# theEricMa/TriplaneTurbo

Measured on AMD Instinct MI355X. Metric: rendered rays/sec (fwd+bwd) at 256x256 rays x 128 samples, higher is better.
Workload: dtype f32 (fp32-grade: exact 3-piece fp16 operand split, 6 x v_mfma_f32_32x32x16_f16 per k-step, fp32 accumulation)

## Files before the change

### triplaneturbo_amd/csrc/tt_backward.hip

```cpp
#include "tt_backward_common.h"

struct BwdGeoParams {
    const float* packed;
    MlpPtrs w;
    const float* rays_o;
    const float* rays_d;
    const float* t_starts;
    const float* t_ends;
    tt_render_cfg cfg;
    TileGeom geom;
    long long n_items;
    int* queue;
    const float* ws;
    int n_copies;
    float* grad_packed;
    MlpGradPtrs grads;
    unsigned long long* phase_cycles;
};

#define GEO_SCRATCH_FLOATS (2 * 64 * XS)
#define GOFF_W1T LDS_GEO_FLOATS
#define GOFF_W2T (GOFF_W1T + IMG16_FLOATS(32, 64))
#define LDS_GEO16_FLOATS (GOFF_W2T + IMG16_FLOATS(64, 64))
#define GLO_W1 LDS_GEO16_FLOATS
#define GLO_W2 (GLO_W1 + LO16_FLOATS(64, 32))
#define GLO_W1T (GLO_W2 + LO16_FLOATS(64, 64))
#define GLO_W2T (GLO_W1T + LO16_FLOATS(32, 64))
#define LDS_GEO3_FLOATS (GLO_W2T + LO16_FLOATS(64, 64))
template <int PREC>
struct GeoWFloats {
    static constexpr int value = PREC == PREC_S3 ? LDS_GEO3_FLOATS : LDS_GEO16_FLOATS;
};

template <int PREC, bool WG16, bool STATS = false>
__global__ __launch_bounds__(256, 1) void k_decode_bwd_geo(BwdGeoParams p) {
    constexpr bool EXACT = PREC == PREC_F32;
    constexpr int NT = PrecNT<PREC>::value, WF = GeoWFloats<PREC>::value;
    __shared__ __attribute__((aligned(16))) float L[WF + 4 * (GEO_SCRATCH_FLOATS + SCATTER_TAG_INTS)];
    {
        MlpPtrs w = p.w;
        stage_weights<PREC, 64, 32>(L + OFF_W1, L + GLO_W1, w.w1);
        stage_weights<PREC, 64, 64>(L + OFF_W2, L + GLO_W2, w.w2);
        lds_load_matrix(L + OFF_W3, w.w3, 1, 64, 64);
        stage_weights_t<PREC, 64, 32>(L + GOFF_W1T, L + GLO_W1T, w.w1);
        stage_weights_t<PREC, 64, 64>(L + GOFF_W2T, L + GLO_W2T, w.w2);
    }
    const tt_render_cfg& cfg = p.cfg;
    float sA1 = 1.f, sU = 1.f, sA2 = 1.f, sV = 1.f;
    if (WG16) {
        const unsigned* bnd = reinterpret_cast<const unsigned*>(p.queue) + TT_SLOT_BOUNDS;
        const float Pm = __builtin_bit_cast(float, bnd[TT_BOUND_PLANES]), Sb = __builtin_bit_cast(float, bnd[TT_BOUND_UP0]),
                    Gb = __builtin_bit_cast(float, bnd[TT_BOUND_UP1]);
        unsigned* word = reinterpret_cast<unsigned*>(L + WF);
        const int t = threadIdx.x;
        float w1row = 0.f, a1col = 0.f, w3abs = 0.f;
        if (t < 64) {
            for (int c = 0; c < 32; ++c) w1row += __builtin_fabsf(p.w.w1[t * 32 + c]);
            for (int r = 0; r < 64; ++r) a1col += __builtin_fabsf(p.w.w2[r * 64 + t]) * __builtin_fabsf(p.w.w3[r]);
            w3abs = __builtin_fabsf(p.w.w3[t]);
        }
        const float W1max = block_max(w1row, word), A1max = block_max(a1col, word), A2max = block_max(w3abs, word);
        const float jsum = (0.5f * cfg.plane_w + 0.5f * cfg.plane_h) / cfg.radius;
        const float Fmax = 3.f * Pm, H1max = W1max * Fmax;
        const float Umax = Fmax * (Sb + 2.f * jsum * Gb), QBmax = Fmax * 2.f * jsum * Gb;
        const float Vmax = Sb * H1max + W1max * QBmax;
        sA1 = wg16_scale(A1max);
        sU = wg16_scale(Umax);
        sA2 = wg16_scale(A2max);
        sV = wg16_scale(Vmax);
    }
    const TileGeom& tg = p.geom;
    const int lane = threadIdx.x & 63, i = lane & 31, hi = lane >> 5, wave_in_blk = threadIdx.x >> 6;
    float* Xs = L + WF + wave_in_blk * (GEO_SCRATCH_FLOATS + SCATTER_TAG_INTS);
    float* Ys = Xs + 64 * XS;
    int* tags = reinterpret_cast<int*>(Ys + 64 * XS);
    scatter_init_tags(tags, lane);
    __syncthreads();
    const int S = cfg.n_samples;
    ItemQueue iq = item_queue(p.queue, tg.n_blocks, tg.n_chunks, tg.unit);
    const int H = cfg.plane_h, W = cfg.plane_w;
    const size_t HW = (size_t)H * W;
    const size_t plane_stride = 6 * HW * TT_C;
    const float ju = 0.5f * W / cfg.radius, jv = 0.5f * H / cfg.radius;
    float* const grad_out =
        p.grad_packed + (size_t)(blockIdx.x % (unsigned)p.n_copies) * cfg.n_prompts * plane_stride;
    const unsigned grad_bytes =
        TT_DBG(cfg.flags, TT_DBG_NO_ATOMICS) ? 0u : (unsigned)(cfg.n_prompts * plane_stride * sizeof(float));

    const TileStats st = STATS ? tile_stats(cfg.stats) : TileStats{nullptr};
    f32x16 accW1[2][1] = {{ZERO16}, {ZERO16}};
    f32x16 accW2[2][2] = {{ZERO16, ZERO16}, {ZERO16, ZERO16}};
    float accw3 = 0.f;
#ifdef TT_TUNING
    unsigned long long ph_acc[20] = {0, 0, 0, 0, 0, 0, 0, 0, 0, 0, 0, 0, 0, 0, 0, 0, 0, 0, 0, 0};
    unsigned long long ph_t = __builtin_amdgcn_s_memtime();
#endif

#pragma nounroll
    for (;;) {
        long long b;
        int ck;
        if (!item_pop(iq, tg.order, tg.n_chunks, b, ck)) break;
        if (b >= tg.n_blocks) continue;
        bool ray_ok;
        const long long ray = tile_ray(tg, b, i, ray_ok);
        const float ray_okf = tt_opaque(ray_ok ? 1.f : 0.f);
        const int ks = i % tg.sb;
        const int view = (int)(ray / cfg.rays_per_view);
        const size_t pofs = (size_t)(view / cfg.views_per_prompt) * plane_stride;
        const float ox = p.rays_o[ray * 3 + 0], oy = p.rays_o[ray * 3 + 1], oz = p.rays_o[ray * 3 + 2];
        const float dx = p.rays_d ? p.rays_d[ray * 3 + 0] : 0.f, dy = p.rays_d ? p.rays_d[ray * 3 + 1] : 0.f,
                    dz = p.rays_d ? p.rays_d[ray * 3 + 2] : 0.f;
        const int s_end = (ck + 1) * tg.chunk < S ? (ck + 1) * tg.chunk : S;
        struct StepIn {
            f32x4 up;
            float ts, te;
        };
        auto load_step = [&](int sb0) {
            StepIn r;
            const int si = sb0 + ks;
            const long long sidx = ray * S + (si < S ? si : S - 1);
            r.up = *reinterpret_cast<const f32x4*>(p.ws + sidx * 4);
            r.ts = p.rays_d ? p.t_starts[sidx] : 0.f;
            r.te = p.rays_d ? p.t_ends[sidx] : 0.f;
            return r;
        };
        StepIn in = load_step(ck * tg.chunk), in_next;
#pragma nounroll
        for (int sb0 = ck * tg.chunk; sb0 < s_end; sb0 += tg.sb, in = in_next) {
            in_next = load_step(sb0 + tg.sb);
            const int si = sb0 + ks;
            const bool rvalid = ray_ok && si < s_end;
            const float vf = ray_okf * (si < s_end ? 1.f : 0.f);
            const float sbar = in.up[0] * vf, gbx = in.up[1] * vf, gby = in.up[2] * vf, gbz = in.up[3] * vf;
            tile_stat(st, TT_STAT_VISITED);
            TT_PHASE(0);
            if (!__any(!((__builtin_fabsf(sbar) + __builtin_fabsf(gbx)) + (__builtin_fabsf(gby) + __builtin_fabsf(gbz)) <=
                         cfg.skip_eps_geo)))
                continue;
            float tm, px, py, pz;
            sample_position(ox, oy, oz, dx, dy, dz, in.ts, in.te, tm, px, py, pz);
            const float X = scale_coord(px, cfg.radius), Y = scale_coord(py, cfg.radius),
                        Z = scale_coord(pz, cfg.radius);
            float f[16], u[16];
            unsigned pmask;
            const bool any = __any(gather_geo_bwd_c(p.packed, (unsigned)(pofs / TT_C), H, W, X, Y, Z, rvalid, sbar, gbx,
                                                    gby, gbz, ju, jv, lane, Xs, f, u, pmask,
                                                    tile_stat_ptr(st, TT_STAT_INBOUNDS)));
            TT_PHASE(1);
            if (!any) continue;
            const bool one = single_plane(pmask);
            tile_stat_executed(st, one);
            float h1[32], h2[32], a2[32], a1[32], q[16], u1, u2;
            mvx<PREC, 64, 32, true>(L + OFF_W1, L + GLO_W1, f, h1, i, hi, 1.f, &u1);
#pragma unroll
            for (int r = 0; r < 32; ++r) h1[r] = fmaxf(h1[r], 0.f);
            mvx<PREC, 64, 64, true>(L + OFF_W2, L + GLO_W2, h1, h2, i, hi, u1, &u2);
#pragma unroll
            for (int r = 0; r < 32; ++r) h2[r] = fmaxf(h2[r], 0.f);
#pragma unroll
            for (int g = 0; g < 8; ++g) {
                f32x4 w3 = *reinterpret_cast<const f32x4*>(L + OFF_W3 + 8 * g + 4 * hi);
#pragma unroll
                for (int e2 = 0; e2 < 4; ++e2) a2[4 * g + e2] = h2[4 * g + e2] > 0.f ? w3[e2] : 0.f;
            }
            Split16<64, PAIR_SEQ, NT> a2s, a1s;
            float ua1 = 1.f;
            if (WG16) {
                split16_vec<64, PAIR_SEQ, NT>(a2, sA2, a2s);
                mv16_pre<64, 64, true, NT>(L + GOFF_W2T, a2s, 1.f / sA2, a1, i, hi, &ua1, L + GLO_W2T);
            } else {
                mvtx_copy<PREC, 64, 64, 64>(L + GOFF_W2T, L + GLO_W2T, L + OFF_W2, a2, a1, i, hi);
            }
#pragma unroll
            for (int r = 0; r < 32; ++r) a1[r] = h1[r] > 0.f ? a1[r] : 0.f;
            if (WG16) {
                split16_vec<64, PAIR_SEQ, NT>(a1, sA1 * ua1, a1s);
                mv16_pre<32, 64, false, NT>(L + GOFF_W1T, a1s, 1.f / sA1, q, i, hi, nullptr, L + GLO_W1T);
            } else {
                mvtx_copy<PREC, 32, 64, 32>(L + GOFF_W1T, L + GLO_W1T, L + OFF_W1, a1, q, i, hi);
            }
            TT_PHASE(3);
            {
                float qb[16];
#pragma unroll
                for (int r = 0; r < 16; ++r) qb[r] = fmaf(-sbar, f[r], u[r]);
                const bool region = WG16 ? true : cfg.flags >= 0;
                const bool do_wgrad = region && !TT_DBG(cfg.flags, TT_DBG_NO_WGRAD);
                if (do_wgrad) {
                    if (WG16) {
                        stage_rows16_pre<64>(Xs, a1s, i, hi);
                        stage_rows16<32>(Ys, u, i, hi, sU);
                        wgrad16<64, 32>(accW1, Xs, Ys, i, hi);
                    } else {
                        stage_rows<64>(Xs, a1, i, hi);
                        stage_rows<32>(Ys, u, i, hi);
                        wgrad<64, 32>(accW1, Xs, Ys, i, hi);
                    }
                }
                TT_PHASE(7);
                float t1[32];
                mvx<PREC, 64, 32>(L + OFF_W1, L + GLO_W1, qb, t1, i, hi);
#pragma unroll
                for (int r = 0; r < 32; ++r) t1[r] = h1[r] > 0.f ? t1[r] : 0.f;
                float v[32];
#pragma unroll
                for (int r = 0; r < 32; ++r) v[r] = fmaf(sbar * u1, h1[r], t1[r]);
                TT_PHASE(4);
                if (do_wgrad) {
                    if (WG16) {
                        stage_rows16_pre<64>(Xs, a2s, i, hi);
                        stage_rows16<64>(Ys, v, i, hi, sV);
                        wgrad16<64, 64>(accW2, Xs, Ys, i, hi);
                    } else {
                        stage_rows<64>(Xs, a2, i, hi);
                        stage_rows<64>(Ys, v, i, hi);
                        wgrad<64, 64>(accW2, Xs, Ys, i, hi);
                    }
                }
                TT_PHASE(8);
                float t2[32];
                mvx<PREC, 64, 64>(L + OFF_W2, L + GLO_W2, t1, t2, i, hi);
#pragma unroll
                for (int r = 0; r < 32; ++r) t2[r] = fmaf(sbar * u2, h2[r], h2[r] > 0.f ? t2[r] : 0.f);
                stage_rows<64>(Xs, t2, i, hi);
                accw3 += rowsum32(Xs, lane);
                TT_PHASE(5);
                if (region && !TT_DBG(cfg.flags, TT_DBG_NO_SCATTER)) {
                    scatter_clear<EXACT>(Xs, lane);
                    float* Qs = Xs + SCATTER_M_FLOATS;
                    TT_PHASE(9);
                    const int tex0 = (int)(pofs / TT_C);
                    auto prep = [&](int pl, PlaneRefs& refs) {
                        Corners c;
                        float coef[4];
                        geo_corner_coefs(pl, H, W, X, Y, Z, rvalid, sbar, gbx, gby, gbz, ju, jv, c, coef);
                        int aoff[4];
#pragma unroll
                        for (int q4 = 0; q4 < 4; ++q4) aoff[q4] = tex0 + (int)(pl * HW) + c.off[q4];
                        refs = plane_refs<!EXACT>(coef, aoff, c.hs, hi);
#pragma unroll
                        for (int r = 0; r < 16; ++r) Qs[i * 33 + LIDX(r, hi)] = q[r] * refs.qs;
                    };
#ifdef TT_TUNING
                    unsigned long long* const sc_st = ph_acc + 14;
#else
                    unsigned long long* const sc_st = nullptr;
#endif
                    if (one)
                        scatter_one_plane<EXACT>(grad_out, grad_bytes, Qs, Xs, tags, Qs + 32 * 33, i, hi,
                                                 single_plane_index(pmask), prep, sc_st);
                    else
                        scatter_planes<EXACT>(grad_out, grad_bytes, Qs, Xs, tags, Qs + 32 * 33, i, hi, prep, sc_st);
                    TT_PHASE(10);
                }
            }
        }
    }
#ifdef TT_TUNING
    TT_PHASE(11);
    if (p.phase_cycles && lane == 0)
        for (int k = 0; k < 20; ++k) atomicAdd(p.phase_cycles + 20 + k, ph_acc[k]);
#endif
    __syncthreads();
    int parity = 0;
    flush_wgrad_reduced<64, 32>(L, parity, accW1, p.grads.w1, wave_in_blk, lane, 1.f / sA1, 1.f / sU);
    flush_wgrad_reduced<64, 64>(L, parity, accW2, p.grads.w2, wave_in_blk, lane, 1.f / sA2, 1.f / sV);
    atomicAdd(p.grads.w3 + lane, accw3);
    tile_stats_flush(st);
}

#ifdef TT_TUNING
unsigned long long* g_phase_cycles = nullptr;
extern "C" int tt_tuning_phase_cycles(unsigned long long* out40) {
    if (!g_phase_cycles) {
        if (hipMalloc((void**)&g_phase_cycles, 40 * sizeof(unsigned long long)) != hipSuccess) return -4;
        if (hipMemset(g_phase_cycles, 0, 40 * sizeof(unsigned long long)) != hipSuccess) return -4;
    }
    if (hipDeviceSynchronize() != hipSuccess) return -4;
    if (out40 && hipMemcpy(out40, g_phase_cycles, 40 * sizeof(unsigned long long), hipMemcpyDeviceToHost) != hipSuccess)
        return -4;
    return hipMemset(g_phase_cycles, 0, 40 * sizeof(unsigned long long)) == hipSuccess ? 0 : -4;
}
#endif
static void launch_bwd_geo(const BwdGeoParams& p0, long long blocks, hipStream_t s) {
    BwdGeoParams p = p0;
#ifdef TT_TUNING
    p.phase_cycles = g_phase_cycles;
#else
    p.phase_cycles = nullptr;
#endif
    if (use_wg16(p.cfg)) {
        unsigned* bnd = reinterpret_cast<unsigned*>(p.queue) + TT_SLOT_BOUNDS;
        launch_planes_bound(p.packed, p.cfg, 0, bnd + TT_BOUND_PLANES, s);
        const long long n = p.cfg.n_rays * p.cfg.n_samples;
        hipLaunchKernelGGL(k_absmax4, dim3(absmax_blocks(n), 1), dim3(256), 0, s, reinterpret_cast<const f32x4*>(p.ws), n, n,
                           bnd + TT_BOUND_UP0, bnd + TT_BOUND_UP1);
    }
    tt_dispatch_prec(tt_prec_of_r(p.cfg.flags), [&](auto P) {
        constexpr int PREC = decltype(P)::value;
        constexpr bool WG16 = PREC != PREC_F32;
        if (p.cfg.stats)
            hipLaunchKernelGGL((k_decode_bwd_geo<PREC, WG16, true>), dim3((unsigned)blocks), dim3(256), 0, s, p);
        else
            hipLaunchKernelGGL((k_decode_bwd_geo<PREC, WG16>), dim3((unsigned)blocks), dim3(256), 0, s, p);
    });
}

extern "C" int tt_render_bwd_geo(const float* packed, const tt_mlp_weights* w, const float* rays_o,
                                 const float* rays_d, const float* t_starts, const float* t_ends,
                                 const tt_render_cfg* cfg, const float* opacity, const float* depth,
                                 const float* trans, const float* sdf, const float* sdf_grad, const float* features,
                                 const float* g_opacity, const float* g_depth, const float* g_rgb_fg,
                                 const float* g_z_variance, const float* g_normal_acc, const float* g_weights,
                                 const float* g_sdf, const float* g_sdf_grad, float* g_inv_std_rays, float* workspace,
                                 float* grad_packed, const tt_mlp_grads* grads, void* stream) {
    int st = tt_validate_cfg(cfg);
    if (st != TT_OK) return st;
    if (!packed || !w || !rays_o || !rays_d || !t_starts || !t_ends || !opacity || !depth || !trans || !sdf ||
        !sdf_grad || !features || !workspace || !grad_packed || !grads)
        return TT_ERR_BAD_ARG;
    if (!w->w1 || !w->w2 || !w->w3 || !grads->w1 || !grads->w2 || !grads->w3) return TT_ERR_BAD_ARG;
    if (grad_buffer_too_large(cfg)) return TT_ERR_UNSUPPORTED;
    int cus = tt_num_cus();
    if (cus <= 0) return TT_ERR_DEVICE;
    hipStream_t s = (hipStream_t)stream;
    st = tt_launch_march_bwd(rays_d, t_starts, t_ends, cfg, sdf, sdf_grad, features, trans, opacity, depth, g_opacity,
                             g_depth, g_rgb_fg, g_z_variance, g_normal_acc, g_weights, g_sdf, g_sdf_grad, g_inv_std_rays,
                             workspace, s);
    if (st != TT_OK) return st;
    BwdGeoParams p;
    tt_fill_rays(p, packed, w, rays_o, rays_d, t_starts, t_ends, *cfg);
    p.cfg.flags |= debug_flags();
    p.ws = workspace;
    p.grad_packed = grad_packed;
    p.n_copies = cfg->grad_copies > 0 ? cfg->grad_copies : 1;
    p.grads = to_gptrs(grads);
    st = tt_plan_queue(cfg, 4LL * cus, s, &p.geom, &p.n_items, &p.queue);
    if (st != TT_OK) return st;
    launch_bwd_geo(p, tt_persistent_blocks(p.n_items, cus, 4), s);
    return tt_check_launch();
}

__global__ void k_interleave_ws(const float* __restrict__ g_sdf, const float* __restrict__ g_sdf_grad,
                                float* __restrict__ ws, long long n) {
    const long long i = (long long)blockIdx.x * blockDim.x + threadIdx.x;
    if (i >= n) return;
    f32x4 o = {g_sdf ? g_sdf[i] : 0.f, g_sdf_grad ? g_sdf_grad[i * 3 + 0] : 0.f,
               g_sdf_grad ? g_sdf_grad[i * 3 + 1] : 0.f, g_sdf_grad ? g_sdf_grad[i * 3 + 2] : 0.f};
    *reinterpret_cast<f32x4*>(ws + i * 4) = o;
}

extern "C" int tt_points_bwd_geo(const float* packed, const tt_mlp_weights* w, const float* points, int32_t n_batch,
                                 int64_t n_points, int32_t n_prompts, int32_t views_per_prompt, int32_t plane_h,
                                 int32_t plane_w, float radius, float sdf_bias_radius, int32_t flags,
                                 const float* g_sdf, const float* g_sdf_grad, float* workspace, float* grad_packed,
                                 const tt_mlp_grads* grads, void* stream) {
    tt_render_cfg cfg;
    int st = points_cfg(&cfg, n_batch, n_points, n_prompts, views_per_prompt, plane_h, plane_w, radius,
                        sdf_bias_radius, 1, flags);
    if (st != TT_OK) return st;
    if (grad_buffer_too_large(&cfg)) return TT_ERR_UNSUPPORTED;
    if (!packed || !w || !points || !workspace || !grad_packed || !grads || (!g_sdf && !g_sdf_grad))
        return TT_ERR_BAD_ARG;
    if (!w->w1 || !w->w2 || !w->w3 || !grads->w1 || !grads->w2 || !grads->w3) return TT_ERR_BAD_ARG;
    int cus = tt_num_cus();
    if (cus <= 0) return TT_ERR_DEVICE;
    hipStream_t s = (hipStream_t)stream;
    const long long n = cfg.n_rays;
    hipLaunchKernelGGL(k_interleave_ws, dim3((unsigned)((n + 255) / 256)), dim3(256), 0, s, g_sdf, g_sdf_grad,
                       workspace, n);
    st = tt_check_launch();
    if (st != TT_OK) return st;
    BwdGeoParams p;
    tt_fill_rays(p, packed, w, points, nullptr, nullptr, nullptr, cfg);
    p.ws = workspace;
    p.grad_packed = grad_packed;
    p.n_copies = 1;
    p.grads = to_gptrs(grads);
    st = tt_plan_queue(&cfg, 4LL * cus, s, &p.geom, &p.n_items, &p.queue);
    if (st != TT_OK) return st;
    launch_bwd_geo(p, tt_persistent_blocks(p.n_items, cus, 4), s);
    return tt_check_launch();
}
```

### triplaneturbo_amd/csrc/tt_backward_common.h

```cpp
#pragma once
#include "tt_device.h"
#include "tt_mfma16.h"
#include "tt_alpha.h"
#include "tt_launch.h"
#include <type_traits>

typedef int i32x4 __attribute__((ext_vector_type(4)));

#ifdef TT_TUNING
#define TT_PHASE(k)                                              \
    do {                                                         \
        __builtin_amdgcn_sched_barrier(0);                       \
        const unsigned long long t_now = __builtin_amdgcn_s_memtime(); \
        ph_acc[k] += t_now - ph_t;                               \
        ph_t = t_now;                                            \
        __builtin_amdgcn_sched_barrier(0);                       \
    } while (0)
#else
#define TT_PHASE(k) \
    do {            \
    } while (0)
#endif
#define XS 36

template <int N>
__device__ __forceinline__ void stage_rows(float* S, const float (&v)[N / 2], int j, int hi) {
#pragma unroll
    for (int r = 0; r < N / 2; ++r) S[LIDX(r, hi) * XS + j] = v[r];
}
template <int N, int OFF, int TOT>
__device__ __forceinline__ void stage_rows_sub(float* S, const float (&v)[TOT], int j, int hi) {
#pragma unroll
    for (int r = 0; r < N / 2; ++r) S[LIDX(r, hi) * XS + j] = v[OFF + r];
}

template <int NX, int NY>
__device__ __forceinline__ void wgrad(f32x16 (&acc)[NX / 32][NY / 32], const float* Xs, const float* Ys, int i,
                                      int hi) {
#pragma unroll
    for (int t4 = 0; t4 < 4; ++t4) {
        f32x4 xa[NX / 32], yb[NY / 32];
#pragma unroll
        for (int m = 0; m < NX / 32; ++m)
            xa[m] = *reinterpret_cast<const f32x4*>(Xs + (32 * m + i) * XS + 16 * hi + 4 * t4);
#pragma unroll
        for (int n = 0; n < NY / 32; ++n)
            yb[n] = *reinterpret_cast<const f32x4*>(Ys + (32 * n + i) * XS + 16 * hi + 4 * t4);
#pragma unroll
        for (int k = 0; k < 4; ++k)
#pragma unroll
            for (int m = 0; m < NX / 32; ++m)
#pragma unroll
                for (int n = 0; n < NY / 32; ++n)
                    acc[m][n] = __builtin_amdgcn_mfma_f32_32x32x2f32(xa[m][k], yb[n][k], acc[m][n], 0, 0, 0);
    }
}

template <int NY>
__device__ __forceinline__ void wgrad_row(f32x16 (&acc)[NY / 32], const float* Xs, const float* Ys, int i, int hi) {
#pragma unroll
    for (int t4 = 0; t4 < 4; ++t4) {
        f32x4 yb[NY / 32];
        const f32x4 xa = *reinterpret_cast<const f32x4*>(Xs + i * XS + 16 * hi + 4 * t4);
#pragma unroll
        for (int n = 0; n < NY / 32; ++n)
            yb[n] = *reinterpret_cast<const f32x4*>(Ys + (32 * n + i) * XS + 16 * hi + 4 * t4);
#pragma unroll
        for (int k = 0; k < 4; ++k)
#pragma unroll
            for (int n = 0; n < NY / 32; ++n)
                acc[n] = __builtin_amdgcn_mfma_f32_32x32x2f32(xa[k], yb[n][k], acc[n], 0, 0, 0);
    }
}

__device__ __forceinline__ float rowsum32(const float* Xs, int lane) {
    float s = 0.f;
#pragma unroll
    for (int g = 0; g < 8; ++g) {
        f32x4 a = *reinterpret_cast<const f32x4*>(Xs + lane * XS + 4 * g);
        s += (a[0] + a[1]) + (a[2] + a[3]);
    }
    return s;
}

typedef unsigned u32x4 __attribute__((ext_vector_type(4)));

__device__ __forceinline__ float wg16_scale(float bound) {
    int E = (int)(__builtin_bit_cast(unsigned, bound * 1.0001f) >> 23) & 0xff;
    E = E < 16 ? 16 : (E > 240 ? 240 : E);
    return __builtin_bit_cast(float, (unsigned)(268 - E) << 23);
}
__device__ __forceinline__ unsigned wg16_pack(float x) {
    unsigned out;
    float r;
    asm("v_cvt_pk_f16_f32 %0, %2, 0\n\t"
        "v_fma_mix_f32 %1, %2, 1.0, -%0 op_sel_hi:[0,0,1]\n\t"
        "v_cvt_pk_f16_f32 %0, %2, %1"
        : "=&v"(out), "=&v"(r)
        : "v"(x));
    return out;
}
template <int N>
__device__ __forceinline__ void stage_rows16(float* S, const float (&v)[N / 2], int j, int hi, float sc) {
    unsigned* U = reinterpret_cast<unsigned*>(S);
#pragma unroll
    for (int r = 0; r < N / 2; ++r) U[LIDX(r, hi) * XS + j] = wg16_pack(v[r] * sc);
}
template <int N, int OFF, int TOT>
__device__ __forceinline__ void stage_rows16_sub(float* S, const float (&v)[TOT], int j, int hi, float sc) {
    unsigned* U = reinterpret_cast<unsigned*>(S);
#pragma unroll
    for (int r = 0; r < N / 2; ++r) U[LIDX(r, hi) * XS + j] = wg16_pack(v[OFF + r] * sc);
}
template <int N, int PAIR, int NT>
__device__ __forceinline__ void stage_rows16_pre(float* S, const Split16<N, PAIR, NT>& v, int j, int hi) {
    unsigned* U = reinterpret_cast<unsigned*>(S);
#pragma unroll
    for (int t = 0; t < N / 4; ++t) {
        U[LIDX(pair_reg<PAIR>(t, 0), hi) * XS + j] = __builtin_amdgcn_perm(v.l[t], v.h[t], 0x05040100u);
        U[LIDX(pair_reg<PAIR>(t, 1), hi) * XS + j] = __builtin_amdgcn_perm(v.l[t], v.h[t], 0x07060302u);
    }
}
__device__ __forceinline__ h8_t wg16_frag(const float* S, int row, int t, int hi) {
    return __builtin_bit_cast(h8_t, *reinterpret_cast<const u32x4*>(S + row * XS + 8 * t + 4 * hi));
}
__device__ __forceinline__ h8_t wg16_swap(h8_t v) {
    u32x4 u = __builtin_bit_cast(u32x4, v);
#pragma unroll
    for (int d = 0; d < 4; ++d) u[d] = __builtin_amdgcn_alignbit(u[d], u[d], 16);
    return __builtin_bit_cast(h8_t, u);
}
template <int NX, int NY>
__device__ __forceinline__ void wgrad16(f32x16 (&acc)[NX / 32][NY / 32], const float* Xs, const float* Ys, int i,
                                        int hi) {
#pragma unroll
    for (int t = 0; t < 4; ++t) {
        h8_t xa[NX / 32], yb[NY / 32], ys[NY / 32];
#pragma unroll
        for (int m = 0; m < NX / 32; ++m) xa[m] = wg16_frag(Xs, 32 * m + i, t, hi);
#pragma unroll
        for (int n = 0; n < NY / 32; ++n) {
            yb[n] = wg16_frag(Ys, 32 * n + i, t, hi);
            ys[n] = wg16_swap(yb[n]);
        }
#pragma unroll
        for (int m = 0; m < NX / 32; ++m)
#pragma unroll
            for (int n = 0; n < NY / 32; ++n)
                acc[m][n] = __builtin_amdgcn_mfma_f32_32x32x16_f16(xa[m], yb[n], acc[m][n], 0, 0, 0);
#pragma unroll
        for (int m = 0; m < NX / 32; ++m)
#pragma unroll
            for (int n = 0; n < NY / 32; ++n)
                acc[m][n] = __builtin_amdgcn_mfma_f32_32x32x16_f16(xa[m], ys[n], acc[m][n], 0, 0, 0);
    }
}
template <int NY>
__device__ __forceinline__ void wgrad16_row(f32x16 (&acc)[NY / 32], const float* Xs, const float* Ys, int i, int hi) {
#pragma unroll
    for (int t = 0; t < 4; ++t) {
        const h8_t xa = wg16_frag(Xs, i, t, hi);
        h8_t yb[NY / 32], ys[NY / 32];
#pragma unroll
        for (int n = 0; n < NY / 32; ++n) {
            yb[n] = wg16_frag(Ys, 32 * n + i, t, hi);
            ys[n] = wg16_swap(yb[n]);
        }
#pragma unroll
        for (int n = 0; n < NY / 32; ++n) acc[n] = __builtin_amdgcn_mfma_f32_32x32x16_f16(xa, yb[n], acc[n], 0, 0, 0);
#pragma unroll
        for (int n = 0; n < NY / 32; ++n) acc[n] = __builtin_amdgcn_mfma_f32_32x32x16_f16(xa, ys[n], acc[n], 0, 0, 0);
    }
}

__device__ __forceinline__ float block_max(float v, unsigned* word) {
    __syncthreads();
    if (threadIdx.x == 0) *word = 0u;
    __syncthreads();
#pragma unroll
    for (int o = 32; o > 0; o >>= 1) v = fmaxf(v, __shfl_xor(v, o));
    if ((threadIdx.x & 63) == 0) atomicMax(word, __builtin_bit_cast(unsigned, v));
    __syncthreads();
    const float r = __builtin_bit_cast(float, *word);
    __syncthreads();
    return r;
}

template <int NX, int NY>
__device__ __forceinline__ void flush_wgrad(const f32x16 (&acc)[NX / 32][NY / 32], float* __restrict__ dst, int i,
                                            int hi, float ux = 1.f, float uy = 1.f) {
#pragma unroll
    for (int m = 0; m < NX / 32; ++m)
#pragma unroll
        for (int n = 0; n < NY / 32; ++n)
#pragma unroll
            for (int r = 0; r < 16; ++r)
                atomicAdd(dst + (32 * m + LIDX(r, hi)) * NY + 32 * n + i, (acc[m][n][r] * ux) * uy);
}

template <class Addr>
__device__ __forceinline__ void flush_tile_reduced(float* R, int parity, const f32x16& acc, int wave, int lane,
                                                   float ux, float uy, Addr addr) {
    float* B = R + parity * 4096;
#pragma unroll
    for (int r = 0; r < 16; ++r) B[(wave * 16 + r) * 64 + lane] = (acc[r] * ux) * uy;
    __syncthreads();
#pragma unroll
    for (int q = 0; q < 4; ++q) {
        const int r = 4 * wave + q;
        const float v = (B[r * 64 + lane] + B[(16 + r) * 64 + lane]) + (B[(32 + r) * 64 + lane] + B[(48 + r) * 64 + lane]);
        atomicAdd(addr(r), v);
    }
}
template <int NX, int NY>
__device__ __forceinline__ void flush_wgrad_reduced(float* R, int& parity, const f32x16 (&acc)[NX / 32][NY / 32],
                                                    float* __restrict__ dst, int wave, int lane, float ux, float uy) {
    const int i = lane & 31, hi = lane >> 5;
#pragma unroll
    for (int m = 0; m < NX / 32; ++m)
#pragma unroll
        for (int n = 0; n < NY / 32; ++n) {
            flush_tile_reduced(R, parity, acc[m][n], wave, lane, ux, uy,
                               [&](int r) { return dst + (32 * m + LIDX(r, hi)) * NY + 32 * n + i; });
            parity ^= 1;
        }
}

#define ZERO16 \
    { 0.f, 0.f, 0.f, 0.f, 0.f, 0.f, 0.f, 0.f, 0.f, 0.f, 0.f, 0.f, 0.f, 0.f, 0.f, 0.f }

#define MS XS

#define M16_RS 40
#define M16_PLANE (65 * M16_RS)
#define SCATTER_M_FLOATS 2624
template <bool EXACT>
__device__ __forceinline__ void scatter_clear(float* M, int lane) {
    const f32x4 z = {0.f, 0.f, 0.f, 0.f};
    if (EXACT) {
#pragma unroll
        for (int g = 0; g < MS / 4; ++g) *reinterpret_cast<f32x4*>(M + lane * MS + 4 * g) = z;
    } else {
#pragma unroll
        for (int g = 0; g < SCATTER_M_FLOATS / 256; ++g) *reinterpret_cast<f32x4*>(M + (g * 64 + lane) * 4) = z;
        if (lane < (SCATTER_M_FLOATS % 256) / 4)
            *reinterpret_cast<f32x4*>(M + ((SCATTER_M_FLOATS / 256) * 64 + lane) * 4) = z;
    }
}

#define SCATTER_TAG_INTS 160

struct PlaneRefs {
    float c0, c1;
    int o0, o1;
    int h0, h1;
    float qs;
};
template <bool NORM>
__device__ __forceinline__ PlaneRefs plane_refs(const float (&coef)[4], const int (&aoff)[4], const int (&hs)[4],
                                                int hi) {
    PlaneRefs r;
    float cn = 1.f;
    r.qs = 1.f;
    if (NORM) {
        const float m = fmaxf(fmaxf(__builtin_fabsf(coef[0]), __builtin_fabsf(coef[1])),
                              fmaxf(__builtin_fabsf(coef[2]), __builtin_fabsf(coef[3])));
        int E = (int)(__builtin_bit_cast(unsigned, m) >> 23);
        E = E < 16 ? 16 : (E > 240 ? 240 : E);
        cn = __builtin_bit_cast(float, (unsigned)(268 - E) << 23);
        r.qs = __builtin_bit_cast(float, (unsigned)(E - 14) << 23);
    }
    r.c0 = (hi ? coef[2] : coef[0]) * cn;
    r.c1 = (hi ? coef[3] : coef[1]) * cn;
    r.o0 = hi ? aoff[2] : aoff[0];
    r.o1 = hi ? aoff[3] : aoff[1];
    r.h0 = hi ? hs[2] : hs[0];
    r.h1 = hi ? hs[3] : hs[1];
    return r;
}
__device__ __forceinline__ void scatter_init_tags(int* tags, int lane) {
    if (lane < 32) tags[lane] = -2;
}

template <bool EXACT>
__device__ __forceinline__ void m_store(float* M, int row, int i, float c) {
    if (EXACT) {
        M[row * MS + i] = c;
    } else {
        half_t h, l;
        split16(c, h, l);
        half_t* Mh = reinterpret_cast<half_t*>(M);
        Mh[row * M16_RS + i] = h;
        Mh[M16_PLANE + row * M16_RS + i] = l;
    }
}
template <bool EXACT>
__device__ __forceinline__ void m_zero(float* M, int row, int i) {
    if (EXACT) {
        M[row * MS + i] = 0.f;
    } else {
        half_t* Mh = reinterpret_cast<half_t*>(M);
        Mh[row * M16_RS + i] = (half_t)0.f;
        Mh[M16_PLANE + row * M16_RS + i] = (half_t)0.f;
    }
}

__device__ __forceinline__ void scatter_lost(const PlaneRefs& r, bool l0, bool l1, const float* Qs, float* Ls,
                                             __amdgpu_buffer_rsrc_t grsrc, int i, int hi) {
    const float lc0 = l0 ? r.c0 : 0.f, lc1 = l1 ? r.c1 : 0.f;
    const unsigned long long bal = __ballot(__builtin_fabsf(lc0) + __builtin_fabsf(lc1) != 0.f);
    if (bal == 0) return;
    float* Lc = Ls;
    int* Lo = reinterpret_cast<int*>(Ls + 32 * 4);
    Lc[4 * i + 2 * hi] = lc0;
    Lc[4 * i + 2 * hi + 1] = lc1;
    Lo[4 * i + 2 * hi] = r.o0;
    Lo[4 * i + 2 * hi + 1] = r.o1;
    unsigned todo = (unsigned)(bal & 0xffffffffull) | (unsigned)(bal >> 32);
    while (todo) {
        const int s0 = __builtin_ctz(todo);
        todo &= todo - 1;
        int s1 = -1;
        if (todo) {
            s1 = __builtin_ctz(todo);
            todo &= todo - 1;
        }
        const int sidx2 = hi ? s1 : s0;
        if (sidx2 >= 0) {
            const f32x4 c4 = *reinterpret_cast<const f32x4*>(Lc + 4 * sidx2);
            const i32x4 o4 = *reinterpret_cast<const i32x4*>(Lo + 4 * sidx2);
            const float v = Qs[sidx2 * 33 + i];
#pragma unroll
            for (int q = 0; q < 4; ++q) {
                const unsigned tex = c4[q] != 0.f ? (unsigned)o4[q] : ~0u;
                __builtin_amdgcn_raw_ptr_buffer_atomic_fadd_f32(v * c4[q], grsrc, (int)((tex << 7) | (4u * (unsigned)i)),
                                                                0, 0);
            }
        }
    }
}

#define SC2_HT 256
#define SC2_CT 136
#define SC2_INTS (SC2_HT + 2 * SC2_CT + 64)

struct Sc2State {
    int rx0, rx1;
    bool l0, l1;
    int n;
};

__device__ __forceinline__ Sc2State sc2_claim_rank(const PlaneRefs& r, int* htab, int* ct, int* cdump, int* dummy,
                                                   int lane, unsigned long long* st = nullptr) {
    Sc2State s;
    const bool a0 = r.c0 != 0.f, a1 = r.c1 != 0.f;
    int* const e0 = a0 ? htab + r.h0 : dummy;
    int* const e1 = a1 ? htab + r.h1 : dummy;
    const int old0 = atomicCAS(e0, -1, r.o0);
    const int old1 = atomicCAS(e1, -1, r.o1);
    const bool w0 = tt_eq_either(old0, -1, r.o0), w1 = tt_eq_either(old1, -1, r.o1);
    s.l0 = !w0;
    s.l1 = !w1;
    const bool m0 = old0 == -1, m1 = old1 == -1;
    const unsigned long long b0 = __ballot(m0), b1 = __ballot(m1);
    const int n0 = __popcll(b0);
    const int r0 = (int)__builtin_amdgcn_mbcnt_hi((unsigned)(b0 >> 32), __builtin_amdgcn_mbcnt_lo((unsigned)b0, 0u));
    const int r1 = n0 + (int)__builtin_amdgcn_mbcnt_hi((unsigned)(b1 >> 32), __builtin_amdgcn_mbcnt_lo((unsigned)b1, 0u));
    s.n = n0 + __popcll(b1);
    int* const x0 = m0 ? e0 : dummy;
    int* const x1 = m1 ? e1 : dummy;
    *x0 = -2 - r0;
    *x1 = -2 - r1;
    *(m0 ? ct + r0 : cdump + lane) = r.o0;
    *(m1 ? ct + r1 : cdump + lane) = r.o1;
    *(lane < 8 ? ct + s.n + lane : cdump + lane) = -1;
    const int q0 = -2 - *e0, q1 = -2 - *e1;
    *x0 = m0 ? -1 : -2;
    *x1 = m1 ? -1 : -2;
    s.rx0 = w0 ? q0 : 255;
    s.rx1 = w1 ? q1 : 255;
#ifdef TT_TUNING
    if (st) {
        st[0] += __popcll(__ballot(a0)) + __popcll(__ballot(a1));
        st[1] += __popcll(__ballot((s.l0 ? r.c0 : 0.f) != 0.f)) + __popcll(__ballot((s.l1 ? r.c1 : 0.f) != 0.f));
        st[2] += 1;
    }
#endif
    return s;
}
__device__ __forceinline__ int sc2_row_a(int rx) { return rx < 64 ? rx : 64; }
__device__ __forceinline__ int sc2_row_b(int rx) {
    const unsigned d = (unsigned)(rx - 64);
    return (int)(d < 64u ? d : 64u);
}

struct ScA16 {
    h8_t ah[2][2], al[2][2];
};
struct ScB16 {
    float bs[2][8];
    h8_t bh[2], bl[2];
    float bun;
};
struct ScA32 {
    f32x4 a4[2][4];
};
struct ScB32 {
    float bq[16];
};
__device__ __forceinline__ void sc2_load_a(const float* M, int i, int hi, int n, ScA16& A) {
    const half_t* Mh = reinterpret_cast<const half_t*>(M);
#pragma unroll
    for (int m = 0; m < 2; ++m) {
        if (m == 1 && n <= 32) break;
#pragma unroll
        for (int ks = 0; ks < 2; ++ks) {
            const half_t* a = Mh + (32 * m + i) * M16_RS + 16 * ks + 8 * hi;
            A.ah[m][ks] = *reinterpret_cast<const h8_t*>(a);
            A.al[m][ks] = *reinterpret_cast<const h8_t*>(a + M16_PLANE);
        }
    }
}
__device__ __forceinline__ void sc2_load_a(const float* M, int i, int hi, int n, ScA32& A) {
#pragma unroll
    for (int m = 0; m < 2; ++m) {
        if (m == 1 && n <= 32) break;
#pragma unroll
        for (int t4 = 0; t4 < 4; ++t4)
            A.a4[m][t4] = *reinterpret_cast<const f32x4*>(M + (32 * m + i) * MS + 16 * hi + 4 * t4);
    }
}
__device__ __forceinline__ void sc2_load_b(const float* Qs, int i, int hi, ScB16& B) {
#pragma unroll
    for (int ks = 0; ks < 2; ++ks)
#pragma unroll
        for (int j = 0; j < 8; ++j) B.bs[ks][j] = Qs[(16 * ks + 8 * hi + j) * 33 + i];
}
__device__ __forceinline__ void sc2_load_b(const float* Qs, int i, int hi, ScB32& B) {
#pragma unroll
    for (int t = 0; t < 16; ++t) B.bq[t] = Qs[(t + 16 * hi) * 33 + i];
}
__device__ __forceinline__ void sc2_split_b(ScB32&) {}
__device__ __forceinline__ void sc2_split_b(ScB16& B) {
    const float (&bs)[2][8] = B.bs;
    float mx = 0.f;
#pragma unroll
    for (int ks = 0; ks < 2; ++ks)
#pragma unroll
        for (int j = 0; j < 8; ++j) mx = fmaxf(mx, __builtin_fabsf(bs[ks][j]));
    mx = fmaxf(mx, __shfl_xor(mx, 32));
    int E = (int)(__builtin_bit_cast(unsigned, mx) >> 23);
    E = E < 16 ? 16 : (E > 240 ? 240 : E);
    const float bsc = __builtin_bit_cast(float, (unsigned)(268 - E) << 23);
    B.bun = __builtin_bit_cast(float, (unsigned)(E - 14) << 23);
#pragma unroll
    for (int ks = 0; ks < 2; ++ks)
#pragma unroll
        for (int j = 0; j < 4; ++j) {
            const float x0 = bs[ks][2 * j] * bsc, x1 = bs[ks][2 * j + 1] * bsc;
            h2_t ph, pq;
            split_pair(x0, x1, ph, pq);
            B.bh[ks][2 * j] = ph.x;
            B.bh[ks][2 * j + 1] = ph.y;
            B.bl[ks][2 * j] = pq.x;
            B.bl[ks][2 * j + 1] = pq.y;
        }
}
__device__ __forceinline__ void sc2_gemm(const ScA16& A, const ScB16& B, int n, f32x16& acc0, f32x16& acc1) {
    acc0 = f32x16 ZERO16;
#pragma unroll
    for (int ks = 0; ks < 2; ++ks) {
        acc0 = __builtin_amdgcn_mfma_f32_32x32x16_f16(A.ah[0][ks], B.bh[ks], acc0, 0, 0, 0);
        acc0 = __builtin_amdgcn_mfma_f32_32x32x16_f16(A.ah[0][ks], B.bl[ks], acc0, 0, 0, 0);
        acc0 = __builtin_amdgcn_mfma_f32_32x32x16_f16(A.al[0][ks], B.bh[ks], acc0, 0, 0, 0);
    }
#pragma unroll
    for (int r = 0; r < 16; ++r) acc0[r] *= B.bun;
    if (n > 32) {
        acc1 = f32x16 ZERO16;
#pragma unroll
        for (int ks = 0; ks < 2; ++ks) {
            acc1 = __builtin_amdgcn_mfma_f32_32x32x16_f16(A.ah[1][ks], B.bh[ks], acc1, 0, 0, 0);
            acc1 = __builtin_amdgcn_mfma_f32_32x32x16_f16(A.ah[1][ks], B.bl[ks], acc1, 0, 0, 0);
            acc1 = __builtin_amdgcn_mfma_f32_32x32x16_f16(A.al[1][ks], B.bh[ks], acc1, 0, 0, 0);
        }
#pragma unroll
        for (int r = 0; r < 16; ++r) acc1[r] *= B.bun;
    }
}
__device__ __forceinline__ void sc2_gemm(const ScA32& A, const ScB32& B, int n, f32x16& acc0, f32x16& acc1) {
    acc0 = f32x16 ZERO16;
#pragma unroll
    for (int t = 0; t < 16; ++t) acc0 = __builtin_amdgcn_mfma_f32_32x32x2f32(A.a4[0][t >> 2][t & 3], B.bq[t], acc0, 0, 0, 0);
    if (n > 32) {
        acc1 = f32x16 ZERO16;
#pragma unroll
        for (int t = 0; t < 16; ++t) acc1 = __builtin_amdgcn_mfma_f32_32x32x2f32(A.a4[1][t >> 2][t & 3], B.bq[t], acc1, 0, 0, 0);
    }
}
__device__ __forceinline__ void sc2_flush(const f32x16& acc0, const f32x16& acc1, const int* ct, int n,
                                          __amdgpu_buffer_rsrc_t grsrc, unsigned lane_b, int hi) {
#pragma unroll
    for (int g = 0; g < 4; ++g) {
        if (n > 8 * g) {
            const i32x4 k0 = *reinterpret_cast<const i32x4*>(ct + 8 * g + 4 * hi);
#pragma unroll
            for (int e2 = 0; e2 < 4; ++e2)
                __builtin_amdgcn_raw_ptr_buffer_atomic_fadd_f32(acc0[4 * g + e2], grsrc,
                                                                (int)(((unsigned)k0[e2] << 7) | lane_b), 0, 0);
        }
    }
#pragma unroll
    for (int g = 0; g < 4; ++g) {
        if (n > 32 + 8 * g) {
            const i32x4 k1 = *reinterpret_cast<const i32x4*>(ct + 32 + 8 * g + 4 * hi);
#pragma unroll
            for (int e2 = 0; e2 < 4; ++e2)
                __builtin_amdgcn_raw_ptr_buffer_atomic_fadd_f32(acc1[4 * g + e2], grsrc,
                                                                (int)(((unsigned)k1[e2] << 7) | lane_b), 0, 0);
        }
    }
}

template <bool EXACT, class Prep>
__device__ __forceinline__ void scatter_planes(float* __restrict__ grad, unsigned grad_bytes, const float* Qs, float* M,
                                               int* tags, float* Ls, int i, int hi, Prep&& prep,
                                               unsigned long long* st = nullptr) {
    const __amdgpu_buffer_rsrc_t grsrc = __builtin_amdgcn_make_buffer_rsrc(grad, 0, (int)grad_bytes, 0x00020000);
    const unsigned lane_b = 4u * (unsigned)i;
    const int lane = i + 32 * hi;
    int* const dummy = tags + i;
    int* const htab = reinterpret_cast<int*>(Ls + 256);
    int* const ctag = htab + SC2_HT;
    int* const cdump = ctag + 2 * SC2_CT;
    typedef typename std::conditional<EXACT, ScA32, ScA16>::type AOp;
    typedef typename std::conditional<EXACT, ScB32, ScB16>::type BOp;
#ifdef TT_TUNING
    unsigned long long sp_t = __builtin_amdgcn_s_memtime();
#define TT_SUBPHASE(k)                                                    \
    do {                                                                  \
        if (st) {                                                         \
            __builtin_amdgcn_sched_barrier(0);                            \
            const unsigned long long t_now = __builtin_amdgcn_s_memtime(); \
            st[k] += t_now - sp_t;                                        \
            sp_t = t_now;                                                 \
            __builtin_amdgcn_sched_barrier(0);                            \
        }                                                                 \
    } while (0)
#else
#define TT_SUBPHASE(k) \
    do {               \
    } while (0)
#endif
    {
        const i32x4 e4 = {-1, -1, -1, -1};
        *reinterpret_cast<i32x4*>(htab + 4 * lane) = e4;
    }
    PlaneRefs rc, rn;
    Sc2State sc, sn;
    prep(0, rc);
    sc = sc2_claim_rank(rc, htab, ctag, cdump, dummy, lane, st);
    scatter_lost(rc, sc.l0, sc.l1, Qs, Ls, grsrc, i, hi);
    m_store<EXACT>(M, sc2_row_a(sc.rx0), i, rc.c0);
    m_store<EXACT>(M, sc2_row_a(sc.rx1), i, rc.c1);
#pragma unroll
    for (int pl = 0; pl < 3; ++pl) {
        const int* const ct = ctag + SC2_CT * (pl & 1);
        int* const ct_next = ctag + SC2_CT * ((pl + 1) & 1);
        const bool pass_b = sc.n > 64;
        f32x16 acc0, acc1;
        AOp A;
        BOp B;
        sc2_load_a(M, i, hi, sc.n, A);
        m_zero<EXACT>(M, sc2_row_a(sc.rx0), i);
        m_zero<EXACT>(M, sc2_row_a(sc.rx1), i);
        if (pass_b) {
            m_store<EXACT>(M, sc2_row_b(sc.rx0), i, rc.c0);
            m_store<EXACT>(M, sc2_row_b(sc.rx1), i, rc.c1);
        }
        sc2_load_b(Qs, i, hi, B);
        if (pl < 2) prep(pl + 1, rn);
        sc2_split_b(B);
        sc2_gemm(A, B, sc.n, acc0, acc1);
        TT_SUBPHASE(3);
        if (pass_b) {
            sc2_flush(acc0, acc1, ct, 64, grsrc, lane_b, hi);
            sc2_load_a(M, i, hi, sc.n - 64, A);
            m_zero<EXACT>(M, sc2_row_b(sc.rx0), i);
            m_zero<EXACT>(M, sc2_row_b(sc.rx1), i);
        }
        if (pl < 2) sn = sc2_claim_rank(rn, htab, ct_next, cdump, dummy, lane, st);
        TT_SUBPHASE(4);
        if (pass_b) {
            sc2_gemm(A, B, sc.n - 64, acc0, acc1);
            sc2_flush(acc0, acc1, ct + 64, sc.n - 64, grsrc, lane_b, hi);
        } else {
            sc2_flush(acc0, acc1, ct, sc.n, grsrc, lane_b, hi);
        }
        if (pl < 2) {
            scatter_lost(rn, sn.l0, sn.l1, Qs, Ls, grsrc, i, hi);
            m_store<EXACT>(M, sc2_row_a(sn.rx0), i, rn.c0);
            m_store<EXACT>(M, sc2_row_a(sn.rx1), i, rn.c1);
            rc = rn;
            sc = sn;
        }
        TT_SUBPHASE(5);
    }
}

template <bool EXACT, class Prep>
__device__ __forceinline__ void scatter_one_plane(float* __restrict__ grad, unsigned grad_bytes, const float* Qs, float* M,
                                                  int* tags, float* Ls, int i, int hi, int pl, Prep&& prep,
                                                  unsigned long long* st = nullptr) {
    const __amdgpu_buffer_rsrc_t grsrc = __builtin_amdgcn_make_buffer_rsrc(grad, 0, (int)grad_bytes, 0x00020000);
    const unsigned lane_b = 4u * (unsigned)i;
    const int lane = i + 32 * hi;
    int* const dummy = tags + i;
    int* const htab = reinterpret_cast<int*>(Ls + 256);
    int* const ct = htab + SC2_HT;
    int* const cdump = ct + 2 * SC2_CT;
    typename std::conditional<EXACT, ScA32, ScA16>::type A;
    typename std::conditional<EXACT, ScB32, ScB16>::type B;
    {
        const i32x4 e4 = {-1, -1, -1, -1};
        *reinterpret_cast<i32x4*>(htab + 4 * lane) = e4;
    }
    PlaneRefs rc;
    prep(pl, rc);
    const Sc2State sc = sc2_claim_rank(rc, htab, ct, cdump, dummy, lane, st);
    scatter_lost(rc, sc.l0, sc.l1, Qs, Ls, grsrc, i, hi);
    m_store<EXACT>(M, sc2_row_a(sc.rx0), i, rc.c0);
    m_store<EXACT>(M, sc2_row_a(sc.rx1), i, rc.c1);
    const bool pass_b = sc.n > 64;
    f32x16 acc0, acc1;
    sc2_load_a(M, i, hi, sc.n, A);
    m_zero<EXACT>(M, sc2_row_a(sc.rx0), i);
    m_zero<EXACT>(M, sc2_row_a(sc.rx1), i);
    if (pass_b) {
        m_store<EXACT>(M, sc2_row_b(sc.rx0), i, rc.c0);
        m_store<EXACT>(M, sc2_row_b(sc.rx1), i, rc.c1);
    }
    sc2_load_b(Qs, i, hi, B);
    sc2_split_b(B);
    sc2_gemm(A, B, sc.n, acc0, acc1);
    if (pass_b) {
        sc2_flush(acc0, acc1, ct, 64, grsrc, lane_b, hi);
        sc2_load_a(M, i, hi, sc.n - 64, A);
        m_zero<EXACT>(M, sc2_row_b(sc.rx0), i);
        m_zero<EXACT>(M, sc2_row_b(sc.rx1), i);
        sc2_gemm(A, B, sc.n - 64, acc0, acc1);
        sc2_flush(acc0, acc1, ct + 64, sc.n - 64, grsrc, lane_b, hi);
    } else {
        sc2_flush(acc0, acc1, ct, sc.n, grsrc, lane_b, hi);
    }
}

struct BwdTexParams {
    const float* packed;
    MlpPtrs w;
    const float* rays_o;
    const float* rays_d;
    const float* t_starts;
    const float* t_ends;
    tt_render_cfg cfg;
    const float* weights;
    const float* features;
    const float* g_rgb;
    const float* g_features;
    TileGeom geom;
    long long n_items;
    int* queue;
    int n_copies;
    float* grad_packed;
    MlpGradPtrs grads;
    unsigned long long* phase_cycles;
};

#define TEX_W_FLOATS (LDS_W_FLOATS - OFF_V1)
#define TV1 0
#define TV2 (OFF_V2 - OFF_V1)
#define TV3 (OFF_V3 - OFF_V1)
#define TV1T TEX_W_FLOATS
#define TV2T (TV1T + IMG16_FLOATS(96, 64))
#define TEX_W16_FLOATS (TV2T + IMG16_FLOATS(64, 64))
#define TLO_V1 TEX_W_FLOATS
#define TLO_V2 (TLO_V1 + LO16_FLOATS(64, 96))
#define TEX_W3P_FLOATS (TLO_V2 + LO16_FLOATS(64, 64))
template <int PREC>
struct TexWFloats {
    static constexpr int value = PREC == PREC_S3 ? TEX_W3P_FLOATS : TEX_W16_FLOATS;
};

static inline bool grad_buffer_too_large(const tt_render_cfg* cfg) {
    return (long long)cfg->n_prompts * 6 * cfg->plane_h * cfg->plane_w * TT_C * 4 >= (1LL << 32) - 256;
}

#ifdef TT_TUNING
extern unsigned long long* g_phase_cycles;
#endif
static __global__ __launch_bounds__(256) void k_absmax4(const f32x4* __restrict__ x, long long seg4, long long seg_stride4,
                                                 unsigned* __restrict__ out0, unsigned* __restrict__ out1) {
    const f32x4* seg = x + (long long)blockIdx.y * seg_stride4;
    const long long stride = (long long)gridDim.x * blockDim.x;
    float m0 = 0.f, m1 = 0.f;
    long long e = (long long)blockIdx.x * blockDim.x + threadIdx.x;
    for (; e + 3 * stride < seg4; e += 4 * stride) {
        const f32x4 a = seg[e], b = seg[e + stride], c = seg[e + 2 * stride], d = seg[e + 3 * stride];
        m0 = fmaxf(fmaxf(m0, __builtin_fabsf(a[0])), fmaxf(__builtin_fabsf(b[0]), fmaxf(__builtin_fabsf(c[0]), __builtin_fabsf(d[0]))));
#pragma unroll
        for (int k = 1; k < 4; ++k)
            m1 = fmaxf(fmaxf(m1, __builtin_fabsf(a[k])), fmaxf(__builtin_fabsf(b[k]), fmaxf(__builtin_fabsf(c[k]), __builtin_fabsf(d[k]))));
    }
    for (; e < seg4; e += stride) {
        const f32x4 v = seg[e];
        m0 = fmaxf(m0, __builtin_fabsf(v[0]));
        m1 = fmaxf(m1, fmaxf(__builtin_fabsf(v[1]), fmaxf(__builtin_fabsf(v[2]), __builtin_fabsf(v[3]))));
    }
    if (!out1) m0 = fmaxf(m0, m1);
    __shared__ unsigned w[2];
    if (threadIdx.x < 2) w[threadIdx.x] = 0u;
    __syncthreads();
    for (int o = 32; o > 0; o >>= 1) {
        m0 = fmaxf(m0, __shfl_xor(m0, o));
        m1 = fmaxf(m1, __shfl_xor(m1, o));
    }
    if ((threadIdx.x & 63) == 0) {
        atomicMax(&w[0], __builtin_bit_cast(unsigned, m0));
        atomicMax(&w[1], __builtin_bit_cast(unsigned, m1));
    }
    __syncthreads();
    if (threadIdx.x == 0) {
        if (w[0] > __hip_atomic_load(out0, __ATOMIC_RELAXED, __HIP_MEMORY_SCOPE_AGENT)) atomicMax(out0, w[0]);
        if (out1 && w[1] > __hip_atomic_load(out1, __ATOMIC_RELAXED, __HIP_MEMORY_SCOPE_AGENT)) atomicMax(out1, w[1]);
    }
}
static __global__ __launch_bounds__(256) void k_absmax1(const float* __restrict__ x, long long n, unsigned* __restrict__ out) {
    float m = 0.f;
    for (long long e = (long long)blockIdx.x * blockDim.x + threadIdx.x; e < n; e += (long long)gridDim.x * blockDim.x)
        m = fmaxf(m, __builtin_fabsf(x[e]));
    for (int o = 32; o > 0; o >>= 1) m = fmaxf(m, __shfl_xor(m, o));
    __shared__ unsigned w;
    if (threadIdx.x == 0) w = 0u;
    __syncthreads();
    if ((threadIdx.x & 63) == 0) atomicMax(&w, __builtin_bit_cast(unsigned, m));
    __syncthreads();
    if (threadIdx.x == 0 && w > __hip_atomic_load(out, __ATOMIC_RELAXED, __HIP_MEMORY_SCOPE_AGENT)) atomicMax(out, w);
}
static inline unsigned absmax_blocks(long long n) {
    long long b = (n + 256 * 8 - 1) / (256 * 8);
    return (unsigned)(b < 1 ? 1 : (b > 1024 ? 1024 : b));
}
static inline void launch_planes_bound(const float* packed, const tt_render_cfg& cfg, int first_plane, unsigned* out,
                                hipStream_t s) {
    const long long hw4 = (long long)cfg.plane_h * cfg.plane_w * TT_C / 4;
    hipLaunchKernelGGL(k_absmax4, dim3(absmax_blocks(3 * hw4), (unsigned)cfg.n_prompts), dim3(256), 0, s,
                       reinterpret_cast<const f32x4*>(packed) + first_plane * hw4, 3 * hw4, 6 * hw4, out,
                       (unsigned*)nullptr);
}

static inline bool use_wg16(const tt_render_cfg& cfg) { return !(cfg.flags & TT_R_EXACT_F32); }

static inline int points_cfg(tt_render_cfg* c, int32_t n_batch, int64_t n_points, int32_t n_prompts,
                      int32_t views_per_prompt, int32_t plane_h, int32_t plane_w, float radius, float sdf_bias_radius,
                      int32_t grad_copies, int32_t q_flags) {
    if (!tt_points_counts_ok(n_batch, n_points, n_prompts, views_per_prompt, q_flags) || n_points > 0x7fffffffLL)
        return TT_ERR_BAD_ARG;
    c->n_prompts = n_prompts;
    c->views_per_prompt = views_per_prompt;
    c->plane_h = plane_h;
    c->plane_w = plane_w;
    c->rays_per_view = (int32_t)n_points;
    c->n_samples = 1;
    c->n_rays = (int64_t)n_batch * n_points;
    c->radius = radius;
    c->sdf_bias_radius = sdf_bias_radius;
    c->inv_std = 1.f;
    c->inv_std_dev = nullptr;
    c->stats = nullptr;
    c->cos_anneal_ratio = 1.f;
    c->rgb_grad_shrink = 1.f;
    c->flags = (q_flags & TT_Q_EXACT_F32) ? TT_R_EXACT_F32 : ((q_flags & TT_Q_SPLIT2) ? TT_R_SPLIT2 : 0);
    c->image_w = 0;
    c->tile_sb = 1;
    c->tile_chunk = 0;
    c->grad_copies = grad_copies;
    c->skip_eps_tex = 0.f;
    c->skip_eps_geo = 0.f;
    return tt_validate_cfg(c);
}
```

Before: 7.441 million.

## Factor W2/W3 gradients through ReLU mask accumulator, drop per-sample W3 matvec

The per-sample second-layer weight gradient now accumulates mask(h2) ⊗ v instead of a2 ⊗ v, where a2 is the W3-weighted mask. The W3 scale and the W3 gradient are applied once at flush time through a new flush_d_reduced that multiplies by w3 and contracts with W2. This removes the per-sample backward matvec through W2 (t2), its staging and rowsum, and halves the fp16 MFMA count for the W2 wgrad because the 0/1 mask is exact in fp16 and needs no split. The cost is extra work at flush time and reliance on the algebraic identity being exact, including the dropped sbar*u2*h2 term.

```diff
diff --git a/triplaneturbo_amd/csrc/tt_backward.hip b/triplaneturbo_amd/csrc/tt_backward.hip
--- a/triplaneturbo_amd/csrc/tt_backward.hip
+++ b/triplaneturbo_amd/csrc/tt_backward.hip
@@ -90,7 +90,6 @@
     const TileStats st = STATS ? tile_stats(cfg.stats) : TileStats{nullptr};
     f32x16 accW1[2][1] = {{ZERO16}, {ZERO16}};
     f32x16 accW2[2][2] = {{ZERO16, ZERO16}, {ZERO16, ZERO16}};
-    float accw3 = 0.f;
 #ifdef TT_TUNING
     unsigned long long ph_acc[20] = {0, 0, 0, 0, 0, 0, 0, 0, 0, 0, 0, 0, 0, 0, 0, 0, 0, 0, 0, 0};
     unsigned long long ph_t = __builtin_amdgcn_s_memtime();
@@ -151,11 +150,11 @@
             if (!any) continue;
             const bool one = single_plane(pmask);
             tile_stat_executed(st, one);
-            float h1[32], h2[32], a2[32], a1[32], q[16], u1, u2;
+            float h1[32], h2[32], a2[32], a1[32], q[16], u1, uh2;
             mvx<PREC, 64, 32, true>(L + OFF_W1, L + GLO_W1, f, h1, i, hi, 1.f, &u1);
 #pragma unroll
             for (int r = 0; r < 32; ++r) h1[r] = fmaxf(h1[r], 0.f);
-            mvx<PREC, 64, 64, true>(L + OFF_W2, L + GLO_W2, h1, h2, i, hi, u1, &u2);
+            mvx<PREC, 64, 64, true>(L + OFF_W2, L + GLO_W2, h1, h2, i, hi, u1, &uh2);
 #pragma unroll
             for (int r = 0; r < 32; ++r) h2[r] = fmaxf(h2[r], 0.f);
 #pragma unroll
@@ -209,23 +208,16 @@
                 TT_PHASE(4);
                 if (do_wgrad) {
                     if (WG16) {
-                        stage_rows16_pre<64>(Xs, a2s, i, hi);
+                        stage_rows16_mask<64>(Xs, h2, i, hi);
                         stage_rows16<64>(Ys, v, i, hi, sV);
-                        wgrad16<64, 64>(accW2, Xs, Ys, i, hi);
+                        wgrad16_mask<64, 64>(accW2, Xs, Ys, i, hi);
                     } else {
-                        stage_rows<64>(Xs, a2, i, hi);
+                        stage_rows_mask<64>(Xs, h2, i, hi);
                         stage_rows<64>(Ys, v, i, hi);
                         wgrad<64, 64>(accW2, Xs, Ys, i, hi);
                     }
                 }
                 TT_PHASE(8);
-                float t2[32];
-                mvx<PREC, 64, 64>(L + OFF_W2, L + GLO_W2, t1, t2, i, hi);
-#pragma unroll
-                for (int r = 0; r < 32; ++r) t2[r] = fmaf(sbar * u2, h2[r], h2[r] > 0.f ? t2[r] : 0.f);
-                stage_rows<64>(Xs, t2, i, hi);
-                accw3 += rowsum32(Xs, lane);
-                TT_PHASE(5);
                 if (region && !TT_DBG(cfg.flags, TT_DBG_NO_SCATTER)) {
                     scatter_clear<EXACT>(Xs, lane);
                     float* Qs = Xs + SCATTER_M_FLOATS;
@@ -265,8 +257,7 @@
     __syncthreads();
     int parity = 0;
     flush_wgrad_reduced<64, 32>(L, parity, accW1, p.grads.w1, wave_in_blk, lane, 1.f / sA1, 1.f / sU);
-    flush_wgrad_reduced<64, 64>(L, parity, accW2, p.grads.w2, wave_in_blk, lane, 1.f / sA2, 1.f / sV);
-    atomicAdd(p.grads.w3 + lane, accw3);
+    flush_d_reduced<64, 64>(L, parity, accW2, p.w.w2, p.w.w3, p.grads.w2, p.grads.w3, wave_in_blk, lane, 1.f / sV);
     tile_stats_flush(st);
 }
 
diff --git a/triplaneturbo_amd/csrc/tt_backward_common.h b/triplaneturbo_amd/csrc/tt_backward_common.h
--- a/triplaneturbo_amd/csrc/tt_backward_common.h
+++ b/triplaneturbo_amd/csrc/tt_backward_common.h
@@ -33,6 +33,11 @@
 #pragma unroll
     for (int r = 0; r < N / 2; ++r) S[LIDX(r, hi) * XS + j] = v[OFF + r];
 }
+template <int N>
+__device__ __forceinline__ void stage_rows_mask(float* S, const float (&v)[N / 2], int j, int hi) {
+#pragma unroll
+    for (int r = 0; r < N / 2; ++r) S[LIDX(r, hi) * XS + j] = v[r] > 0.f ? 1.f : 0.f;
+}
 
 template <int NX, int NY>
 __device__ __forceinline__ void wgrad(f32x16 (&acc)[NX / 32][NY / 32], const float* Xs, const float* Ys, int i,
@@ -71,16 +76,6 @@
             for (int n = 0; n < NY / 32; ++n)
                 acc[n] = __builtin_amdgcn_mfma_f32_32x32x2f32(xa[k], yb[n][k], acc[n], 0, 0, 0);
     }
-}
-
-__device__ __forceinline__ float rowsum32(const float* Xs, int lane) {
-    float s = 0.f;
-#pragma unroll
-    for (int g = 0; g < 8; ++g) {
-        f32x4 a = *reinterpret_cast<const f32x4*>(Xs + lane * XS + 4 * g);
-        s += (a[0] + a[1]) + (a[2] + a[3]);
-    }
-    return s;
 }
 
 typedef unsigned u32x4 __attribute__((ext_vector_type(4)));
@@ -121,6 +116,12 @@
         U[LIDX(pair_reg<PAIR>(t, 1), hi) * XS + j] = __builtin_amdgcn_perm(v.l[t], v.h[t], 0x07060302u);
     }
 }
+template <int N>
+__device__ __forceinline__ void stage_rows16_mask(float* S, const float (&v)[N / 2], int j, int hi) {
+    unsigned* U = reinterpret_cast<unsigned*>(S);
+#pragma unroll
+    for (int r = 0; r < N / 2; ++r) U[LIDX(r, hi) * XS + j] = v[r] > 0.f ? 0x3C003C00u : 0u;
+}
 __device__ __forceinline__ h8_t wg16_frag(const float* S, int row, int t, int hi) {
     return __builtin_bit_cast(h8_t, *reinterpret_cast<const u32x4*>(S + row * XS + 8 * t + 4 * hi));
 }
@@ -153,6 +154,23 @@
 #pragma unroll
             for (int n = 0; n < NY / 32; ++n)
                 acc[m][n] = __builtin_amdgcn_mfma_f32_32x32x16_f16(xa[m], ys[n], acc[m][n], 0, 0, 0);
+    }
+}
+template <int NX, int NY>
+__device__ __forceinline__ void wgrad16_mask(f32x16 (&acc)[NX / 32][NY / 32], const float* Xs, const float* Ys, int i,
+                                             int hi) {
+#pragma unroll
+    for (int t = 0; t < 4; ++t) {
+        h8_t xa[NX / 32], yb[NY / 32];
+#pragma unroll
+        for (int m = 0; m < NX / 32; ++m) xa[m] = wg16_frag(Xs, 32 * m + i, t, hi);
+#pragma unroll
+        for (int n = 0; n < NY / 32; ++n) yb[n] = wg16_frag(Ys, 32 * n + i, t, hi);
+#pragma unroll
+        for (int m = 0; m < NX / 32; ++m)
+#pragma unroll
+            for (int n = 0; n < NY / 32; ++n)
+                acc[m][n] = __builtin_amdgcn_mfma_f32_32x32x16_f16(xa[m], yb[n], acc[m][n], 0, 0, 0);
     }
 }
 template <int NY>
@@ -224,6 +242,40 @@
                                [&](int r) { return dst + (32 * m + LIDX(r, hi)) * NY + 32 * n + i; });
             parity ^= 1;
         }
+}
+
+template <int NX, int NY>
+__device__ __forceinline__ void flush_d_reduced(float* R, int& parity, const f32x16 (&acc)[NX / 32][NY / 32],
+                                                const float* __restrict__ W, const float* __restrict__ wo,
+                                                float* __restrict__ dW, float* __restrict__ dwo, int wave, int lane,
+                                                float uy) {
+    const int i = lane & 31, hi = lane >> 5;
+#pragma unroll
+    for (int m = 0; m < NX / 32; ++m) {
+        float part[4] = {0.f, 0.f, 0.f, 0.f};
+#pragma unroll
+        for (int n = 0; n < NY / 32; ++n) {
+            float* B = R + parity * 4096;
+#pragma unroll
+            for (int r = 0; r < 16; ++r) B[(wave * 16 + r) * 64 + lane] = acc[m][n][r] * uy;
+            __syncthreads();
+#pragma unroll
+            for (int q = 0; q < 4; ++q) {
+                const int r = 4 * wave + q, at = (32 * m + LIDX(r, hi)) * NY + 32 * n + i;
+                const float d = (B[r * 64 + lane] + B[(16 + r) * 64 + lane]) + (B[(32 + r) * 64 + lane] + B[(48 + r) * 64 + lane]);
+                atomicAdd(dW + at, wo[32 * m + LIDX(r, hi)] * d);
+                part[q] = fmaf(W[at], d, part[q]);
+            }
+            parity ^= 1;
+        }
+#pragma unroll
+        for (int q = 0; q < 4; ++q) {
+            float s = part[q];
+#pragma unroll
+            for (int o = 16; o > 0; o >>= 1) s += __shfl_xor(s, o);
+            if (i == 0) atomicAdd(dwo + 32 * m + LIDX(4 * wave + q, hi), s);
+        }
+    }
 }
 
 #define ZERO16 \
```

Measured after the change: 7.709 million, median of 6. 3.6% higher.
